# moss-lab/ScanFold

Hardware: AMD Instinct MI355X
Metric: windows/sec (W=120, step=1, 100 shuffles) (higher is better)
Workload: dtype int32 (int16 LDS storage) energies; f64 partition function

## Files before the change

### scanfold_amd/csrc/sf_mfe_fast.hip.h

```cpp
#pragma once
#include <type_traits>
#ifdef SF_EMUL
#include <vector>
#endif
#include "sf_energy.h"
#include "sf_pk16.h"

#define SF_FAST_NR 34
#ifndef SF_FAST_TINY_D0
#define SF_FAST_TINY_D0 10
#endif
#define SF_FAST_CHUNK_D0 36
#ifndef SF_FAST_SHORT
#define SF_FAST_SHORT 1
#endif
#ifndef SF_FAST_SHORT_D1
#define SF_FAST_SHORT_D1 18
#endif
#ifndef SF_FAST_SHORT_D2
#define SF_FAST_SHORT_D2 26
#endif
#define SF_FAST_SHORT_D3 32
#ifndef SF_FAST_UNPACK
#define SF_FAST_UNPACK 1
#endif
#ifndef SF_UNP_PB
#define SF_UNP_PB 4
#endif
#define SF_HELP_MERGE_MAXW 118
#define SF_DML_HELPER_BIAS_256 26
#define SF_DML_HELPER_BIAS_W200 50
#define SF_DML_HELPER_BIAS(ng, wt) ((ng) == 256 ? ((wt) == 200 ? SF_DML_HELPER_BIAS_W200 : SF_DML_HELPER_BIAS_256) : 100000)
#define SF_HELP_NB_128 4
#define SF_HELP_NB_128G 8
#define SF_HELP_NB_256 6
#define SF_INF16 30000
#define SF_FAST_THRESH 10000
#define SF_FAST_OVF (-12000)
#define SF_FAST_MAXPARAM 2500
#define SF_FAST_MAXW 256
#define SF_FAST_BIG 60000
#ifndef SF_FAST_WAVES_PER_SIMD
#define SF_FAST_WAVES_PER_SIMD 4
#endif

struct SfFastParams {
  int32_t NIN[32];
  int32_t IL[32];
  int32_t L1N[32];
  int32_t BUL[32];
  int32_t L23;
  int32_t fast_ok;
  int16_t mmI[200], mm1n[200], mm23[200], mmM[200], mmH[200], mmExt[200];
  int16_t stack[64];
  int16_t d5[40], d3[40];
  uint8_t pair[64];
  uint8_t rpair[64];
  int16_t stackT[64], mm23in[200];
  int16_t int11T[8 * 8 * 25], int21a[8 * 8 * 125], int21b[8 * 8 * 125], int22T[8 * 8 * 625];
  int16_t uni[128];
  int16_t uniG[31][128];
};
// ... 252 lines not shown
  if (q < sf_emul_span_lo || q + 2 * n16 > sf_emul_span_hi) {
    fprintf(stderr, "sf_mfe_fast (emulation): read for loop size %d, absent on diagonal %d, outside the rolling tables and their mirror rows (%ld bytes past their end)\n",
            u, d, (long)(q + 2 * n16 - sf_emul_span_hi));
    abort();
  }
  for (int k = 0; k < n16; k++) {
    const int s = sf_emul_shadow[(size_t)(q - sf_emul_span_lo) / 2 + k];
    if (s != 0) {
      fprintf(stderr, "sf_mfe_fast (emulation): read for loop size %d, absent on diagonal %d, finds an entry %s (entry %ld of the rolling tables)\n",
              u, d, s == 1 ? "a diagonal of this fold has written" : "this fold's prologue has not initialised", (long)((q - sf_emul_span_lo) / 2 + k));
      abort();
    }
  }
}
extern "C" int sfemul_absent_check_selftest(int W, int what) {
  const SfFastLayout L = sf_fast_layout(W);
  static std::vector<char> lds;
  lds.assign((size_t)L.total, 0);
  sf_emul_shadow_span(lds.data() + L.off_ci, lds.data() + L.off_tab);
  sf_emul_shadow_set(lds.data() + L.off_ci, (L.off_tab - L.off_ci) / 2, 0);
  if (what == 0) {
    const int16_t *e = (const int16_t *)(lds.data() + L.off_ci) + 3 * (W - 4) + 3;
    sf_emul_check_absent(e, 1, 10, 5);
    sf_emul_shadow_set(e, 1, 1);
    sf_emul_check_absent(e, 1, 10, 5);
  } else {
    sf_emul_check_absent(lds.data() + L.off_tab - 4, 2, 10, 8);
    sf_emul_check_absent(lds.data() + L.off_tab, 2, 10, 8);
  }
  return 0;
}
#define SF_EMUL_WROTE(p, n16) sf_emul_shadow_set((p), (n16), 1)
#define SF_EMUL_ABSENT(CHK, p, n16, d, u) do { if ((CHK) && (u) > (d) - 2 - (SFD_TURN + 1)) sf_emul_check_absent((p), (n16), (d), (u)); } while (0)
#else
#define SF_EMUL_WROTE(p, n16) ((void)0)
#define SF_EMUL_ABSENT(CHK, p, n16, d, u) ((void)0)
#endif

__device__ __forceinline__ void sf_fast_publish_bn(int16_t *w, const int i0, const uint32_t bn) {
  w[0] = (int16_t)sf_lo(bn);
  if (i0 > 0) w[-1] = (int16_t)sf_hi(bn);
  SF_EMUL_WROTE(w, 1);
  if (i0 > 0) SF_EMUL_WROTE(w - 1, 1);
}

enum { SF_SEC_P1 = 1, SF_SEC_HELP = 2, SF_SEC_DML = 4, SF_SEC_FIN = 8, SF_SEC_C0 = 16, SF_SEC_ALL = 31, SF_SEC_PRE = 32,
       SF_SEC_POST = 64 };
struct SfHU {
  short v[27];
};
struct SfPub {
  uint32_t a;
  uint32_t b;
  int tau;
  int type;
};
template <bool G, int WT, int SEC, bool CH = false, bool FOLD = false, int UCAP = SFD_MAXLOOP, int TBLK = 1, bool MGH = false,
          bool UNP = false, bool SHORT = false>
__device__ __forceinline__ void sf_fast_cell(const SfFastCtx &X, const int d, const int i, const bool valid,
                                             const int slot2, const int slotd, uint32_t (&HP)[14], SfHU &HU, int &ovf,
                                             const bool final_fml, const int fnb, int &fpart, int &dec, int &eh, int &e0,
                                             int &dprev, SfPub &pub, const int dml_lo = SFD_TURN + 1,
                                             const int dml_hi = 1 << 20) {
  const SfFastParams *const Fc = FOLD ? X.F : sf_const_base(X.F);
  const int16_t *const ubase = G ? X.uNIN : (CH ? Fc->uniG[sfd_max(sfd_min(d - 2 - (SFD_TURN + 1), 30), 0)] : Fc->uni);
  const int16_t *const uNIN = ubase, *const uIL = ubase + 32, *const uBN = ubase + 64;
#define CBAT(x) X.BN[2 * (x)]
#define C1NAT(x) X.BN[2 * ((x) - 1) + 1]
#define HGET(x) (((x)&1) ? ((int)HP[(x) >> 1] >> 16) : (int)(int16_t)(HP[(x) >> 1] & 0xffffu))
#define HSET(x, v)                                                                                       \
  HP[(x) >> 1] = ((x)&1) ? ((HP[(x) >> 1] & 0x0000ffffu) | ((uint32_t)(v) << 16))                         \
                         : ((HP[(x) >> 1] & 0xffff0000u) | ((uint32_t)(v)&0xffffu))
  const int W = WT ? WT : X.W, RW = W - 4;
  if (!valid) return;
  const int j = i + d, i0 = i - 1;
  const uint8_t *S = X.S;
  const int umax = G ? sfd_min(SFD_MAXLOOP, d - 2 - (SFD_TURN + 1)) : SFD_MAXLOOP;
  const int um = CH ? d - 2 - (SFD_TURN + 1) : SFD_MAXLOOP;
  int type = (SEC & SF_SEC_POST) ? pub.type : (d <= X.maxd ? X.tPair[S[i] * 8 + S[j]] : 0);
  if (!(SEC & SF_SEC_POST) && X.hc.c) {
    type = sf_hc_type_of(X.hc, type, i, j, d <= X.maxd);
    if (type == 7) { type = 0; ovf = 1; }
  }
  const int si1 = S[i + 1], sj1 = S[j - 1];
  if (SEC & SF_SEC_PRE) pub.type = type;
  if ((SEC & SF_SEC_PRE) && type) {
    const int tr = X.tRPair[S[i] * 8 + S[j]];
    const int sp1 = S[i - 1], sq1 = S[j + 1];
    const int tau_in = tr > 2 ? X.TAU : 0;
    int stem, ext;
    if (i > 1 && j < W) { stem = X.tM[SF_TIDX(type, sp1, sq1)]; ext = X.tE[SF_TIDX(type, sp1, sq1)]; }
    else if (i > 1) stem = ext = X.tD5[type * 5 + sp1];
    else if (j < W) stem = ext = X.tD3[type * 5 + sq1];
    else stem = ext = 0;
    pub.a = sf_pk(X.tI[SF_TIDX(tr, sq1, sp1)], X.t1n[SF_TIDX(tr, sq1, sp1)]);
    pub.b = sf_pk(stem + tau_in + X.MLintern, ext + tau_in);
    pub.tau = tau_in;
  }
#define FBASE(dd) (FOLD ? ((dd) <= (W + 3) / 2 ? ((dd)-4) * (W - 3) : (W - 1 - (dd)) * (W - 3) + (dd)-3) \
                        : (((dd)-4) * W - ((dd) * ((dd)-1) / 2 - 6) + (((dd)-4 + (W & 1)) >> 1)))
#define FLEN(dd) (W - (dd) + ((W - (dd)) & 1))
#define ROW(u) ((slot2 - (u) < 0 ? slot2 - (u) + SF_FAST_NR : slot2 - (u)) * RW)
  constexpr bool TBL = !G && TBLK != 0;
  constexpr int UTOP = (!G && UCAP < SFD_MAXLOOP) ? UCAP : SFD_MAXLOOP;
  constexpr bool UNG = !G && !CH;
  const SfFastRows *const Rc = TBL ? sf_const_base(X.R) : X.R;
  const int32_t *const rci_o = Rc->ci_odd[slot2], *const rci_e = Rc->ci_even[slot2];
  const int32_t *const rbn_o = Rc->bn_odd[slot2], *const rbn_e = Rc->bn_even[slot2];
#define ROWB_CI(u) (TBL ? (((u)&1) ? rci_o[(u) >> 1] : rci_e[(u) >> 1]) : 2 * ROW(u))
#define ROWB_BN(u) (TBL ? (((u)&1) ? rbn_o[(u) >> 1] : rbn_e[(u) >> 1]) : 4 * ROW(u))
#define CIROW(u) ((const int16_t *)((const char *)X.CI + ROWB_CI(u)))

  if (SEC & SF_SEC_P1) {
  if (UNP) {
    static_assert(!UNP || (!G && !CH && !FOLD), "the unpacked recurrence exists for the all-sizes code of the narrow kernel only");
    const int32_t *const nin = Fc->NIN;
    static_assert(!UNP || UTOP >= 7, "the unpacked recurrence keeps at least the sizes 6 and 7");
    short r30a = 0, r30b = 0;
    if (UTOP >= 30) {
      const int16_t *row = CIROW(30) + i0;
      SF_EMUL_ABSENT(true, row + 3, 1, d, 30); SF_EMUL_ABSENT(true, row + 29, 1, d, 30);
      r30a = row[3]; r30b = row[29];
    }
    constexpr int PB = SF_UNP_PB;
#pragma unroll
    for (int pb = 12; pb >= 1; pb -= PB) {
      short a3[PB], au[PB], b3[PB], bu[PB];
#pragma unroll
      for (int k = 0; k < PB; k++) {
// ... 304 lines not shown
          uint32_t ggp = sf_pk(32767, 32767);
#pragma unroll
          for (int pp = 1; pp <= 13; pp++)
            if (!CH || um >= 2 * pp + 4) ggp = sf_pkmin(ggp, sf_pkadd(HP[pp], sf_ldw(uIL + 2 * pp + 4)));
          gg = sfd_min(sf_lo(ggp), sf_hi(ggp));
        }
        e = sfd_min(e, gg + X.tI[SF_TIDX(type, si1, sj1)]);
      }
      {
        const int tr = X.tRPair[S[i] * 8 + S[j]];
        const int dml = dprev;
        e = sfd_min(e, dml + X.tM[SF_TIDX(tr, sj1, si1)] + (tr > 2 ? TAU : 0) + X.MLintern + X.MLclosing);
      }
      e0 = e;
    }
  }
  if ((SEC & SF_SEC_DML) && !(SEC & SF_SEC_FIN)) multiloop_split();

  if (!(SEC & SF_SEC_FIN)) return;
  int c = SF_INF16;
  if (type) {
    c = sfd_min(e0, eh);
    if (c < SF_FAST_OVF) ovf = 1;
  }

  const int rbd = slotd * RW + i0;
  int f = SF_FAST_BIG, cx = SF_INF16;
  if (SEC & SF_SEC_POST) {
    X.CI[rbd] = (int16_t)(c + sf_lo(pub.a));
    if (!FOLD && slotd == 0) X.CI[SF_FAST_NR * RW + i0] = (int16_t)(c + sf_lo(pub.a));
    const uint32_t bn = sf_pk(c + pub.tau, c + sf_hi(pub.a));
    sf_fast_publish_bn(X.BN + 2 * rbd, i0, bn);
    if (X.bn_dup && slotd == 0) sf_fast_publish_bn(X.BN + 2 * (SF_FAST_NR * RW + i0), i0, bn);
    f = c + sf_lo(pub.b);
    cx = sfd_min(c + sf_hi(pub.b), SF_INF16);
  } else if (type) {
    const int tr = X.tRPair[S[i] * 8 + S[j]];
    const int sp1 = S[i - 1], sq1 = S[j + 1];
    const int tau_in = tr > 2 ? X.TAU : 0;
    X.CI[rbd] = (int16_t)(c + X.tI[SF_TIDX(tr, sq1, sp1)]);
    if (!FOLD && slotd == 0) X.CI[SF_FAST_NR * RW + i0] = X.CI[rbd];
    const uint32_t bn = sf_pk(c + tau_in, c + X.t1n[SF_TIDX(tr, sq1, sp1)]);
    sf_fast_publish_bn(X.BN + 2 * rbd, i0, bn);
    if (X.bn_dup && slotd == 0) sf_fast_publish_bn(X.BN + 2 * (SF_FAST_NR * RW + i0), i0, bn);
    int stem, ext;
    if (i > 1 && j < W) { stem = X.tM[SF_TIDX(type, sp1, sq1)]; ext = X.tE[SF_TIDX(type, sp1, sq1)]; }
    else if (i > 1) stem = ext = X.tD5[type * 5 + sp1];
    else if (j < W) stem = ext = X.tD3[type * 5 + sq1];
    else stem = ext = 0;
    f = c + stem + tau_in + X.MLintern;
    cx = sfd_min(c + ext + tau_in, SF_INF16);
  } else {
    X.CI[rbd] = SF_INF16; sf_fast_publish_bn(X.BN + 2 * rbd, i0, sf_pk(SF_INF16, SF_INF16));
    if (!FOLD && slotd == 0) X.CI[SF_FAST_NR * RW + i0] = SF_INF16;
    if (X.bn_dup && slotd == 0) sf_fast_publish_bn(X.BN + 2 * (SF_FAST_NR * RW + i0), i0, sf_pk(SF_INF16, SF_INF16));
  }
  SF_EMUL_WROTE(X.CI + rbd, 1);
  if (!FOLD && slotd == 0) SF_EMUL_WROTE(X.CI + SF_FAST_NR * RW + i0, 1);
  X.cg[SF_CGIDX(i, j)] = (int16_t)cx;
  if (final_fml && d > SFD_TURN + 1) f = sfd_min(f, fnb);
  if ((SEC & SF_SEC_DML) && (SEC & SF_SEC_FIN)) multiloop_split();
  f = sfd_min(f, dec);
  dprev = dec > SF_FAST_THRESH ? SF_INF16 : dec;
  fpart = f;
  if (final_fml && f < SF_FAST_OVF) ovf = 1;
  X.fML[FBASE(d) + i0] = (int16_t)(f > SF_FAST_THRESH ? SF_INF16 : f);
#undef ROW
#undef ROWB_CI
#undef ROWB_BN
#undef CIROW
#undef BNROWB
}

__device__ __forceinline__ int sf_wave_min(int v) {
#ifdef SF_EMUL
  return sfemul_wave_min(v);
#else
  v = sfd_min(v, __builtin_amdgcn_update_dpp(v, v, 0xB1, 0xF, 0xF, false));
  v = sfd_min(v, __builtin_amdgcn_update_dpp(v, v, 0x4E, 0xF, 0xF, false));
  v = sfd_min(v, __builtin_amdgcn_update_dpp(v, v, 0x141, 0xF, 0xF, false));
  v = sfd_min(v, __builtin_amdgcn_update_dpp(v, v, 0x140, 0xF, 0xF, false));
  v = sfd_min(v, __builtin_amdgcn_update_dpp(v, v, 0x142, 0xA, 0xF, false));
  v = sfd_min(v, __builtin_amdgcn_update_dpp(v, v, 0x143, 0xC, 0xF, false));
  return __builtin_amdgcn_readlane(v, 63);
#endif
}

__device__ __forceinline__ uint32_t sf_wave_next(uint32_t v) {
#ifdef SF_EMUL
  return __shfl_down(v, 1);
#else
  return (uint32_t)__builtin_amdgcn_update_dpp(0, (int)v, 0x130, 0xF, 0xF, true);
#endif
}

template <int WT, int LGC = 0>
__device__ __forceinline__ int sf_fast_dml2(const SfFastCtx &X, const int d, const int lane, const int i_own, const bool valid) {
  constexpr bool FOLD = false;
  const int W = WT ? WT : X.W;
// ... 264 lines not shown
            }
          }
        }
        }
        load_row(i + PF, cb[k]);
      }
    }
  }
  for (int jf = sfd_max(W - SFD_TURN - 1, 1); jf <= W; jf++) {
    f5prev = sfd_min(f5prev, column_min(jf));
    if (want_trace && lane == 0) f5s[jf] = f5prev;
  }
  SF_WAVE_SYNC();
  const int over = flag[0] || f5prev < SF_FAST_OVF;
  if (lane == 0) {
    out[seq] = f5prev;
    if (over) {
      const int k = atomicAdd(ovf_cnt, 1);
      ovf_list[k] = seq;
    }
  }
  if (db_out && !over && (seq % trace_stride) == 0) {
    int16_t *stI = stack_area;
    int16_t *stJ = stI + W + 8;
    int16_t *stM = stJ + W + 8;
    const int bad = sf_fast_traceback(X, f5s, tExt, lane, stI, stJ, stM, dbL);
    char *dst = db_out + (size_t)(seq / trace_stride) * (W + 1);
    for (int x = lane; x <= W; x += 64) dst[x] = x < W ? dbL[x] : 0;
    if (bad && lane == 0) atomicOr(status, 1);
  }
}

#define SF_DEFER_ROWS_256 3
template <int NQ>
struct SfTrail {
  int F[NQ];
  int f3n;
  int row;
};
template <int NQ>
__device__ __forceinline__ void sf_trail_load(const int16_t *cgp, const int W, const int lane, const int i, int (&c)[NQ]) {
#pragma unroll
  for (int q = 0; q < NQ; q++) {
    const int j = lane + 1 + 64 * q;
    c[q] = (i >= 1 && j <= W && i + SFD_TURN + 1 <= j) ? (int)cgp[SF_CGIDX(i, j)] : SF_INF16;
  }
}
template <int NQ>
__device__ __forceinline__ void sf_trail_row(SfTrail<NQ> &T, const int lane, const int i, const int (&c)[NQ]) {
  if (i < 1) return;
  int m = c[0] + T.F[0];
#pragma unroll
  for (int q = 1; q < NQ; q++) m = sfd_min(m, c[q] + T.F[q]);
  T.f3n = sfd_min(T.f3n, sf_wave_min(m));
  if (i >= 2) {
    const int l = (i - 2) & 63, h = (i - 2) >> 6;
#pragma unroll
    for (int q = 0; q < NQ; q++) T.F[q] = (lane == l && h == q) ? T.f3n : T.F[q];
  }
}
template <int NQ, int NR>
__device__ __forceinline__ void sf_trail_rows(SfTrail<NQ> &T, const int lane, const int nrows, const int (&c)[NR][NQ]) {
#pragma unroll
  for (int k = 0; k < NR; k++)
    if (k < nrows) sf_trail_row<NQ>(T, lane, T.row - k, c[k]);
  T.row -= nrows;
// ... 62 lines not shown
  uint8_t *const hcP = (uint8_t *)hcC + (W + 2), *const hcE = hcP + (W + 2);
  int16_t *const scS = (int16_t *)(smem + Lo.off_hc + (((3 * (W + 2)) + 1) & ~1));
  X.hc.c = (HC && cons_rows) ? hcC : nullptr; X.hc.partner = hcP; X.hc.encl = hcE;
  X.sc = (HC && sc_rows) ? scS : nullptr;
  X.fML = (int16_t *)smem;
  X.CI = (int16_t *)(smem + Lo.off_ci);
  X.C1N = nullptr; X.CB = nullptr;
  X.BN = (int16_t *)(smem + Lo.off_c1n);
#ifdef SF_EMUL
  sf_emul_bn_base = (const char *)X.BN; sf_emul_ci_base = (const char *)X.CI;
  sf_emul_shadow_span((const char *)(smem + Lo.off_ci), (const char *)(smem + Lo.off_tab));
#endif
  X.DMLr = nullptr;
  int16_t *tab = (int16_t *)(smem + Lo.off_tab);
  X.t23 = tab; X.tI = tab + 175 - 25; X.t1n = tab + 325 - 25; X.tM = tab + 475 - 25; X.tH = tab + 625 - 25;
  X.tE = tab + 775 - 25; X.cg_ext = 1;
  X.tStack = tab + 925; X.tD5 = tab + 989; X.tD3 = tab + 1029;
  uint8_t *tPair = (uint8_t *)(tab + 1069);
  X.tPair = tPair;
  uint8_t *tRPair = (uint8_t *)(tab + SF_FAST_TAB_OLD);
  int16_t *t23in = tab + SF_FAST_TAB_OLD + 32;
  X.tRPair = tRPair; X.t23in = t23in;
  int32_t *flag = (int32_t *)(smem + Lo.off_flag);
  uint8_t *S = (uint8_t *)(smem + Lo.off_S);
  X.S = S;
  X.D = D; X.F = F; X.R = Rows; X.W = W; X.fold = FOLD; X.maxd = D->max_pair_dist;
  constexpr bool MERGE = MG && (NG == 128);
  constexpr bool UNPK = SF_FAST_UNPACK && (NG == 128);
  constexpr bool SHORTU = SF_FAST_SHORT && UNPK && !HC;
  static_assert(SF_FAST_TINY_D0 >= 10 && SF_FAST_TINY_D0 <= SF_FAST_SHORT_D1 && SF_FAST_SHORT_D1 <= SF_FAST_SHORT_D2 &&
                SF_FAST_SHORT_D2 <= SF_FAST_SHORT_D3 && SF_FAST_SHORT_D1 >= 14, "SHORT loops: d0 >= 10 (no tabulated hairpin, sizes 0 .. 4 exist), caps >= 7");
  constexpr bool LGLOOPS = MG && (NG == 128);
  constexpr bool ROLE_LOOPS = (NG == 128);
  constexpr int TBLK = WT > 0 ? 1 : (NG == 128 ? (MG ? 2 : 1) : 0);
  X.bn_dup = (NG == 128);
  uint8_t *const cell_list = (MG && W >= SF_HELP_MERGE_MAXW) ? (uint8_t *)((int16_t *)(smem + Lo.off_tab) + 1069 + 32 + 1)
                                                            : (uint8_t *)(smem + Lo.off_list);
  X.TAU = D->P.TerminalAU; X.MLbase = D->P.MLbase; X.MLclosing = D->P.MLclosing; X.MLintern = D->P.MLintern[1];
  int32_t *f5s = (int32_t *)(smem + Lo.off_ci);
  int16_t *tExt = (int16_t *)(smem + Lo.off_ci + (((W + 1) * 4 + 3) & ~3));

  const int tid = threadIdx.x;
  X.cg = cg_all + (size_t)sf_fast_scratch_slot(blockIdx.x, gridDim.x) * SF_CG_ENTRIES(W);
  for (int x = tid; x < 175; x += NT) {
    tab[x] = F->mm23[x];
    if (x < 150) {
      tab[175 + x] = F->mmI[25 + x]; tab[325 + x] = F->mm1n[25 + x]; tab[475 + x] = F->mmM[25 + x];
      tab[625 + x] = F->mmH[25 + x]; tab[775 + x] = F->mmExt[25 + x];
    }
  }
  for (int x = tid; x < 175; x += NT) t23in[x] = F->mm23in[x];
  for (int x = tid; x < 64; x += NT) { tab[925 + x] = F->stackT[x]; tPair[x] = F->pair[x]; tRPair[x] = F->rpair[x]; }
  for (int x = tid; x < 40; x += NT) { tab[989 + x] = F->d5[x]; tab[1029 + x] = F->d3[x]; }

  {
    int16_t *uni = tab + 1069 + 32 + 1;
    X.uNIN = uni;
    for (int x = tid; x < 128; x += NT) uni[x] = F->uni[x];
  }
  const int grp = SF_WAVE_UNIFORM(tid / NG);
  const int tg = tid - grp * NG;
  constexpr int CENTRE = (NG == 256) ? 128 : 32;
  constexpr bool SHARE = SF_DML_HELPER_BIAS(NG, WT) < 10000;
  constexpr bool DML2 = (NG == 128);
  const int OFFs = ((W + 1) >> 1) - CENTRE;
  const int OFF = (NG > 64) ? (OFFs + NG) & (NG - 1) : 0;
// ... 66 lines not shown
    const bool trail_this = defer_on && !(db_out && (seq % trace_stride) == 0);
    if (sweeper) {
#pragma unroll
      for (int q = 0; q < NQ; q++) T.F[q] = 0;
      T.f3n = 0; T.row = trail_this ? W - SFD_TURN - 1 : 0;
    }
    int ovf = 0;
    uint32_t H[14];
    int dprev = SF_INF16;
    int fnb = SF_FAST_BIG;
#pragma unroll
    for (int k = 0; k < 14; k++) H[k] = (uint32_t)SF_INF16 | ((uint32_t)SF_INF16 << 16);

    int slot2 = (SFD_TURN + 1 + grp - 2) % SF_FAST_NR, slotd = (SFD_TURN + 1 + grp) % SF_FAST_NR;
    auto build_list = [&](const int dd0) {
      const int lane = tid & 63;
      const int d1 = dd0 + 1;
      const int iH = ((v - 64) & (NG - 1)) - (dd0 >> 1);
      const bool vA = (dd0 < W) && (iH >= 1) && (iH + dd0 <= W), vB = (d1 < W) && (iH >= 1) && (iH + d1 <= W);
      const int tA = (vA && dd0 <= X.maxd) ? X.tPair[S[iH] * 8 + S[iH + dd0]] : 0;
      const int tB = (vB && d1 <= X.maxd) ? X.tPair[S[iH] * 8 + S[iH + d1]] : 0;
      const unsigned long long mA = __ballot(tA != 0), mB = __ballot(tB != 0);
      const int cA = __popcll(mA);
      uint8_t *list = cell_list + (((dd0 >> 1) & 1) << 7);
      const unsigned long long below = (1ull << lane) - 1ull;
      if (tA) list[__popcll(mA & below)] = (uint8_t)iH;
      if (tB) list[cA + __popcll(mB & below)] = (uint8_t)(iH | 128);
      if (lane == 0) list[127] = (uint8_t)(cA + __popcll(mB));
      if (lane == 0) SF_EMUL_WROTE(list, 64);
    };
    SfHU HU;
    const int grp_wave = grp;
    const bool sweeper_wave = sweeper;
    auto step = [&](const int d0, auto kind_tag, auto role_tag) {
      constexpr SfStep KIND = decltype(kind_tag)::value;
      constexpr SfRole ROLE = decltype(role_tag)::value;
      constexpr bool ROLES = ROLE != SF_ROLE_ALL;
      static_assert(!ROLES || (NG == 128 && KIND >= SF_STEP_SPLIT && KIND <= SF_STEP_SPLIT8), "roles: the narrow kernel's split steps");
      const int grp = ROLES ? (int)(ROLE == SF_ROLE_MAIN_ODD || ROLE == SF_ROLE_HELP_ODD) : grp_wave;
      const bool hwave = ROLES ? ROLE >= SF_ROLE_HELP_EVEN : tg >= 64;
      const bool sweeper = ROLES ? ROLE == SF_ROLE_HELP_ODD : sweeper_wave;
      constexpr int LGC = KIND == SF_STEP_SPLIT16 ? 4 : (KIND == SF_STEP_SPLIT8 ? 3 : (KIND == SF_STEP_SPLIT && LGLOOPS ? 5 : 0));
      constexpr bool DO_G = KIND == SF_STEP_SIZED, DO_CH = KIND == SF_STEP_GUARDED;
      const int d = d0 + grp;
      constexpr bool DO_SH = KIND >= SF_STEP_SHORT_A && KIND <= SF_STEP_SHORT_C;
      constexpr int SHCAP = KIND == SF_STEP_SHORT_A ? SF_FAST_SHORT_D1 - 7 : (KIND == SF_STEP_SHORT_B ? SF_FAST_SHORT_D2 - 7 : SFD_MAXLOOP);
      if (!ROLES && d0 == SFD_TURN + 1 + 2 && tid == 0) *next_slot = fetched;
      if (!ROLES && d0 == SFD_TURN + 1 + 4) next_seq = SF_WAVE_UNIFORM(*next_slot);
      constexpr bool split = KIND >= SF_STEP_SPLIT;
      constexpr bool narrow = KIND == SF_STEP_NARROW;
      if (NARROW && d0 == narrow_d0) {
        uint32_t *const xa = (uint32_t *)X.BN;
        const int RWc = W - 4;
        if (tg >= 96 && tg < 160) {
#pragma unroll
          for (int k = 0; k < 14; k++) xa[(grp * 16 + k) * RWc + 100 + (tg - 96)] = H[k];
          xa[(grp * 16 + 14) * RWc + 100 + (tg - 96)] = (uint32_t)dprev;
          xa[(grp * 16 + 15) * RWc + 100 + (tg - 96)] = (uint32_t)fnb;
        }
        __syncthreads();
        if (tg >= 64 && tg < 128) {
#pragma unroll
          for (int k = 0; k < 14; k++) H[k] = xa[(grp * 16 + k) * RWc + 100 + (tg - 64)];
          dprev = (int)xa[(grp * 16 + 14) * RWc + 100 + (tg - 64)];
          fnb = (int)xa[(grp * 16 + 15) * RWc + 100 + (tg - 64)];
        }
        __syncthreads();
      }
      const bool helper = split && (NG == 256 ? (narrow ? tg < 64 : (tg < 64 || tg >= 192)) : hwave);
      const int vh = NG == 256 ? (narrow ? v + 96 : (tg < 64 ? v + 64 : v - 64)) : v - 64;
      const int vm = narrow ? ((v + 32) & (NG - 1)) : v;
      constexpr bool DML4 = NARROW && (WT == 200);
      const bool dmlw = DML4 && narrow && tg >= 128;
      const int vd = tg >= 192 ? v - 96 : v - 32;
      const int i = (NARROW && !DML4 && narrow && tg >= 128) ? -1
                    : ((dmlw ? (vd & (NG - 1)) : (helper ? (vh & (NG - 1)) : vm)) - (d >> 1));
      const int dml_terms = d - 2 * SFD_TURN - 2;
      const int dml_cut = d - SFD_TURN - 1 - sfd_max(sfd_min(dml_terms / 2 - SF_DML_HELPER_BIAS(NG, WT), dml_terms), 0);
      const bool valid = (d < W) && (i >= 1) && (i + d <= W);
      int fpart = SF_FAST_BIG;
      int dec = SF_FAST_BIG, eh = SF_FAST_BIG, e0 = SF_FAST_BIG;
      SfPub pub;
      pub.a = pub.b = 0; pub.tau = 0; pub.type = 0;
      int dc[DROWS][NQ];
      const bool sweep_now = defer_on && sweeper && split && T.row > 0;
      const int sweep_rows = sweep_now ? sfd_max(sfd_min(defer_rows, T.row - (W - d0)), 0) : 0;
      if (sweep_now) {
#pragma unroll
        for (int k = 0; k < DROWS; k++)
          if (k < sweep_rows) sf_trail_load<NQ>(X.cg, W, tid & 63, T.row - k, dc[k]);
      }
      if (__ballot(valid)) {
        if (DO_G && d0 < 8) sf_fast_cell<true, WT, SF_SEC_ALL, false, FOLD, 1>(X, d, i, valid, slot2, slotd, H, HU, ovf, grp == 0, fnb, fpart, dec, eh, e0, dprev, pub);
        else if (DO_G && d0 < SF_FAST_TINY_D0) sf_fast_cell<true, WT, SF_SEC_ALL, false, FOLD, 5>(X, d, i, valid, slot2, slotd, H, HU, ovf, grp == 0, fnb, fpart, dec, eh, e0, dprev, pub);
        else if (DO_CH && d0 < SF_FAST_CHUNK_D0) sf_fast_cell<false, WT, SF_SEC_ALL, true, FOLD, SFD_MAXLOOP, TBLK>(X, d, i, valid, slot2, slotd, H, HU, ovf, grp == 0, fnb, fpart, dec, eh, e0, dprev, pub);
        else if (DO_SH) sf_fast_cell<false, WT, SF_SEC_ALL, false, FOLD, SHORTU ? SHCAP : SFD_MAXLOOP, TBLK, false, SHORTU, SHORTU>(X, d, i, valid, slot2, slotd, H, HU, ovf, grp == 0, fnb, fpart, dec, eh, e0, dprev, pub);
        else if (!split) sf_fast_cell<false, WT, SF_SEC_ALL, false, FOLD, SFD_MAXLOOP, TBLK, false, UNPK && KIND == SF_STEP_UNSPLIT>(X, d, i, valid, slot2, slotd, H, HU, ovf, grp == 0, fnb, fpart, dec, eh, e0, dprev, pub);
        else if (DML4 && narrow) {
          const int nmain = dml_terms / 5, cA = SFD_TURN + 1 + nmain, cB = cA + (dml_terms - nmain + 1) / 2;
          uint32_t *const xa = (uint32_t *)X.BN;
          if (dmlw) {
            const bool wB = tg >= 192;
            sf_fast_cell<false, WT, SF_SEC_DML, false, FOLD, SFD_MAXLOOP, TBLK>(X, d, i, valid, slot2, slotd, H, HU, ovf, false, fnb, fpart, dec, eh, e0, dprev, pub, wB ? cB : cA, wB ? (1 << 20) : cB - 1);
            if (valid) xa[(grp * 16 + (wB ? 1 : 0)) * (W - 4) + 100 + (tg & 63)] = (uint32_t)sfd_min(dec, 32000);
          } else if (!helper) {
            sf_fast_cell<false, WT, SF_SEC_P1 | SF_SEC_C0 | SF_SEC_DML | SF_SEC_PRE, false, FOLD, SFD_MAXLOOP, TBLK>(X, d, i, valid, slot2, slotd, H, HU, ovf, grp == 0, fnb, fpart, dec, eh, e0, dprev, pub, SFD_TURN + 1, cA - 1);
          } else {
            sf_fast_cell<false, WT, SF_SEC_HELP, false, FOLD, SFD_MAXLOOP, TBLK>(X, d, i, valid, slot2, slotd, H, HU, ovf, grp == 0, fnb, fpart, dec, eh, e0, dprev, pub);
            if (valid) X.BN[2 * (slotd * (W - 4) + i - 1)] = (int16_t)sfd_min(eh, 32000);
          }
        }
        else if (!helper) {
          if (SHARE) sf_fast_cell<false, WT, SF_SEC_P1 | SF_SEC_C0 | SF_SEC_DML | SF_SEC_PRE, false, FOLD, SFD_MAXLOOP, TBLK>(X, d, i, valid, slot2, slotd, H, HU, ovf, grp == 0, fnb, fpart, dec, eh, e0, dprev, pub, SFD_TURN + 1, dml_cut - 1);
          else {
            static_assert(SHARE || DML2, "a main wave either shares the multiloop split with its helpers (NG = 256) or runs it two cells per lane (NG = 128)");
            dec = sf_fast_dml2<WT, LGC>(X, d, tid & 63, i, valid);
            sf_fast_cell<false, WT, SF_SEC_P1 | SF_SEC_C0 | SF_SEC_PRE, false, FOLD, SFD_MAXLOOP, TBLK, false, UNPK && split>(X, d, i, valid, slot2, slotd, H, HU, ovf, grp == 0, fnb, fpart, dec, eh, e0, dprev, pub);
          }
        } else if (MERGE) {
          const int lane = tid & 63;
          const uint8_t *list = cell_list + (((d0 >> 1) & 1) << 7);
          const int cT = SF_WAVE_UNIFORM((int)list[127]);
          const int e = (grp << 6) + lane;
          if (SF_WAVE_UNIFORM(cT > (grp << 6))) {
            const bool vC = e < cT;
            const int ent = vC ? list[e] : 1;
            const int g = ent >> 7, iC = ent & 127;
            const int s2 = slot2 - grp < 0 ? slot2 - grp + SF_FAST_NR : slot2 - grp;
            const int sd0 = slotd - grp < 0 ? slotd - grp + SF_FAST_NR : slotd - grp;
            const int sd1 = sd0 + 1 >= SF_FAST_NR ? 0 : sd0 + 1;
            SfFastCtx Xh = X;
            Xh.BN = X.BN + 2 * g * (W - 4);
            sf_fast_cell<false, WT, SF_SEC_HELP, false, FOLD, SFD_MAXLOOP, TBLK, true>(Xh, d0 + g, iC, vC, s2, sd0, H, HU, ovf, false, fnb, fpart, dec, eh, e0, dprev, pub);
            if (vC) { X.BN[2 * ((g ? sd1 : sd0) * (W - 4) + iC - 1)] = (int16_t)sfd_min(eh, 32000); SF_EMUL_WROTE(X.BN + 2 * ((g ? sd1 : sd0) * (W - 4) + iC - 1), 1); }
          }
        } else {
          if (SHARE) {
            sf_fast_cell<false, WT, SF_SEC_HELP | SF_SEC_DML, false, FOLD, SFD_MAXLOOP, TBLK>(X, d, i, valid, slot2, slotd, H, HU, ovf, grp == 0, fnb, fpart, dec, eh, e0, dprev, pub, dml_cut);
            if (valid) {
              X.BN[2 * (slotd * (W - 4) + i - 1)] = (int16_t)sfd_min(eh, 32000);
              X.CI[slotd * (W - 4) + i - 1] = (int16_t)sfd_min(dec, 32000);
            }
          } else {
            sf_fast_cell<false, WT, SF_SEC_HELP, false, FOLD, SFD_MAXLOOP, TBLK>(X, d, i, valid, slot2, slotd, H, HU, ovf, grp == 0, fnb, fpart, dec, eh, e0, dprev, pub);
            if (valid) { X.BN[2 * (slotd * (W - 4) + i - 1)] = (int16_t)sfd_min(eh, 32000); SF_EMUL_WROTE(X.BN + 2 * (slotd * (W - 4) + i - 1), 1); }
          }
        }
      }
      if (sweep_now && sweep_rows > 0) sf_trail_rows<NQ, DROWS>(T, tid & 63, sweep_rows, dc);
      if (MERGE && grp == 1 && hwave && (ROLES || d0 + 2 >= split_d0) && d0 + 2 < W) build_list(d0 + 2);
      if (split) {
        __syncthreads();
        if (!helper && !dmlw && __ballot(valid)) {
          if (valid) {
            eh = X.BN[2 * (slotd * (W - 4) + i - 1)];
            if (DML4 && narrow) {
              const uint32_t *const xa = (const uint32_t *)X.BN;
              dec = sfd_min(dec, sfd_min((int)xa[(grp * 16) * (W - 4) + 100 + (tg & 63)], (int)xa[(grp * 16 + 1) * (W - 4) + 100 + (tg & 63)]));
            } else if (SHARE) dec = sfd_min(dec, (int)X.CI[slotd * (W - 4) + i - 1]);
          }
          sf_fast_cell<false, WT, SF_SEC_FIN | SF_SEC_POST, false, FOLD, SFD_MAXLOOP, TBLK>(X, d, i, valid, slot2, slotd, H, HU, ovf, grp == 0, fnb, fpart, dec, eh, e0, dprev, pub);
        }
      }
      __syncthreads();
      if (grp == 0 && valid && !helper && !dmlw) {
        const int d1 = d0 + 1;
        const int16_t *pd = X.fML + FBASE(d1), *pe = X.fML + FBASE(d0);
        const bool ex0 = i + d1 <= W, ex1 = i >= 2;
        const int ia = i - 1, ib = ex1 ? i - 2 : 0;
        const int p0 = pd[ia], p1 = pd[ib], q0 = pe[i], q1 = pe[ia], q2 = pe[ib];
        const int v0 = sfd_min(p0, sfd_min(q0, q1) + X.MLbase), v1 = sfd_min(p1, sfd_min(q1, q2) + X.MLbase);
        if ((ex0 && v0 < SF_FAST_OVF) || (ex1 && v1 < SF_FAST_OVF)) ovf = 1;
        const int g0 = (ex0 && v0 <= SF_FAST_THRESH) ? v0 : SF_INF16, g1 = (ex1 && v1 <= SF_FAST_THRESH) ? v1 : SF_INF16;
        if (ex0) X.fML[FBASE(d1) + ia] = (int16_t)g0;
        fnb = sfd_min(g0, g1) + X.MLbase;
      }
      slot2 += 2; if (slot2 >= SF_FAST_NR) slot2 -= SF_FAST_NR;
      slotd += 2; if (slotd >= SF_FAST_NR) slotd -= SF_FAST_NR;
    };
    {
      int d0 = SFD_TURN + 1;
      constexpr SfRoleTag<SF_ROLE_ALL> all_roles{};
      auto unpack_state = [&]() {
#pragma unroll
        for (int x = 0; x < 27; x++) HU.v[x] = (short)((x & 1) ? (H[x >> 1] >> 16) : (H[x >> 1] & 0xffffu));
      };
      for (; d0 < SF_FAST_TINY_D0 && d0 < W; d0 += 2) step(d0, SfStepTag<SF_STEP_SIZED>{}, all_roles);
      if constexpr (SHORTU) {
        unpack_state();
        for (; d0 < SF_FAST_SHORT_D1 && d0 < W; d0 += 2) step(d0, SfStepTag<SF_STEP_SHORT_A>{}, all_roles);
        for (; d0 < SF_FAST_SHORT_D2 && d0 < W; d0 += 2) step(d0, SfStepTag<SF_STEP_SHORT_B>{}, all_roles);
        for (; d0 < SF_FAST_SHORT_D3 && d0 < W; d0 += 2) step(d0, SfStepTag<SF_STEP_SHORT_C>{}, all_roles);
      } else {
        for (; d0 < SF_FAST_CHUNK_D0 && d0 < W; d0 += 2) step(d0, SfStepTag<SF_STEP_GUARDED>{}, all_roles);
        if constexpr (UNPK) unpack_state();
      }
      for (; d0 < split_d0 && d0 < W; d0 += 2) step(d0, SfStepTag<SF_STEP_UNSPLIT>{}, all_roles);
      auto split_loops = [&](auto role_tag) {
        if constexpr (LGLOOPS) {
          for (; d0 < W - 30 && d0 < W; d0 += 2) step(d0, SfStepTag<SF_STEP_SPLIT>{}, role_tag);
          for (; d0 < W - 14 && d0 < W; d0 += 2) step(d0, SfStepTag<SF_STEP_SPLIT16>{}, role_tag);
          for (; d0 < W; d0 += 2) step(d0, SfStepTag<SF_STEP_SPLIT8>{}, role_tag);
        }
        for (; d0 < W; d0 += 2) step(d0, SfStepTag<SF_STEP_SPLIT>{}, role_tag);
      };
      if constexpr (ROLE_LOOPS) {
        const int wave = SF_WAVE_UNIFORM(tid >> 6);
        if (wave == 0) split_loops(SfRoleTag<SF_ROLE_MAIN_EVEN>{});
        else if (wave == 2) split_loops(SfRoleTag<SF_ROLE_MAIN_ODD>{});
        else if (wave == 1) split_loops(SfRoleTag<SF_ROLE_HELP_EVEN>{});
        else split_loops(SfRoleTag<SF_ROLE_HELP_ODD>{});
        if (wave != 3) {
#pragma unroll
          for (int q = 0; q < NQ; q++) T.F[q] = 0;
          T.f3n = 0; T.row = 0;
        }
      } else {
        for (; d0 < (NARROW ? narrow_d0 : W) && d0 < W; d0 += 2) step(d0, SfStepTag<SF_STEP_SPLIT>{}, all_roles);
      }
      if constexpr (NARROW)
        for (; d0 < W; d0 += 2) step(d0, SfStepTag<SF_STEP_NARROW>{}, all_roles);
    }

    if (ovf) flag[0] = 1;
    if (trail_this) {
      __syncthreads();
      if (sweeper) {
        while (T.row >= 1) {
          int tc[4][NQ];
#pragma unroll
          for (int k = 0; k < 4; k++) sf_trail_load<NQ>(X.cg, W, tid & 63, T.row - k, tc[k]);
// ... 80 lines not shown
```

Baseline: 47210.

## Move exterior-loop term lookups to helper waves and carry fML diagonal base

In the split diagonal loops with NG=128, helper waves now compute the pair's stem/ext and interior terms (SF_SEC_TERMS) and hand them to the main wave through LDS scratch in BN/CI/fML. This takes table lookups off the main wave's critical path. The fML diagonal base offset is now carried incrementally in a scalar instead of being recomputed with the quadratic FBASE formula each step. For W=120, sweep row counts are specialised per loop kind. The cost is extra LDS writes and reads for the hand-over, and a dependence on enough free room in the BN rows.

```diff
diff --git a/scanfold_amd/csrc/sf_mfe_fast.hip.h b/scanfold_amd/csrc/sf_mfe_fast.hip.h
--- a/scanfold_amd/csrc/sf_mfe_fast.hip.h
+++ b/scanfold_amd/csrc/sf_mfe_fast.hip.h
@@ -28,6 +28,12 @@
 #define SF_UNP_PB 4
 #endif
 #define SF_HELP_MERGE_MAXW 118
+#ifndef SF_FAST_HELPER_TERMS
+#define SF_FAST_HELPER_TERMS 1
+#endif
+#ifndef SF_FAST_FBASE_CARRY
+#define SF_FAST_FBASE_CARRY 1
+#endif
 #define SF_DML_HELPER_BIAS_256 26
 #define SF_DML_HELPER_BIAS_W200 50
 #define SF_DML_HELPER_BIAS(ng, wt) ((ng) == 256 ? ((wt) == 200 ? SF_DML_HELPER_BIAS_W200 : SF_DML_HELPER_BIAS_256) : 100000)
@@ -346,9 +352,13 @@
 }
 #define SF_EMUL_WROTE(p, n16) sf_emul_shadow_set((p), (n16), 1)
 #define SF_EMUL_ABSENT(CHK, p, n16, d, u) do { if ((CHK) && (u) > (d) - 2 - (SFD_TURN + 1)) sf_emul_check_absent((p), (n16), (d), (u)); } while (0)
+#define SF_LOCKSTEP() ((void)__ballot(1))
+#define SF_PIN_S(x) ((void)0)
 #else
 #define SF_EMUL_WROTE(p, n16) ((void)0)
 #define SF_EMUL_ABSENT(CHK, p, n16, d, u) ((void)0)
+#define SF_LOCKSTEP() ((void)0)
+#define SF_PIN_S(x) asm volatile("" : "+s"(x))
 #endif
 
 __device__ __forceinline__ void sf_fast_publish_bn(int16_t *w, const int i0, const uint32_t bn) {
@@ -359,7 +369,7 @@
 }
 
 enum { SF_SEC_P1 = 1, SF_SEC_HELP = 2, SF_SEC_DML = 4, SF_SEC_FIN = 8, SF_SEC_C0 = 16, SF_SEC_ALL = 31, SF_SEC_PRE = 32,
-       SF_SEC_POST = 64 };
+       SF_SEC_POST = 64, SF_SEC_TERMS = 128, SF_SEC_TYPE = 256, SF_SEC_XTERMS = 512, SF_SEC_FB = 1024 };
 struct SfHU {
   short v[27];
 };
@@ -368,6 +378,7 @@
   uint32_t b;
   int tau;
   int type;
+  int stem, ext;
 };
 template <bool G, int WT, int SEC, bool CH = false, bool FOLD = false, int UCAP = SFD_MAXLOOP, int TBLK = 1, bool MGH = false,
           bool UNP = false, bool SHORT = false>
@@ -375,7 +386,7 @@
                                              const int slot2, const int slotd, uint32_t (&HP)[14], SfHU &HU, int &ovf,
                                              const bool final_fml, const int fnb, int &fpart, int &dec, int &eh, int &e0,
                                              int &dprev, SfPub &pub, const int dml_lo = SFD_TURN + 1,
-                                             const int dml_hi = 1 << 20) {
+                                             const int dml_hi = 1 << 20, const int fbd = 0) {
   const SfFastParams *const Fc = FOLD ? X.F : sf_const_base(X.F);
   const int16_t *const ubase = G ? X.uNIN : (CH ? Fc->uniG[sfd_max(sfd_min(d - 2 - (SFD_TURN + 1), 30), 0)] : Fc->uni);
   const int16_t *const uNIN = ubase, *const uIL = ubase + 32, *const uBN = ubase + 64;
@@ -397,18 +408,27 @@
     if (type == 7) { type = 0; ovf = 1; }
   }
   const int si1 = S[i + 1], sj1 = S[j - 1];
-  if (SEC & SF_SEC_PRE) pub.type = type;
-  if ((SEC & SF_SEC_PRE) && type) {
+  if (SEC & (SF_SEC_PRE | SF_SEC_TYPE)) pub.type = type;
+  if (SEC & SF_SEC_TYPE) pub.tau = type > 2 ? X.TAU : 0;
+  if ((SEC & (SF_SEC_PRE | SF_SEC_TERMS)) && type) {
     const int tr = X.tRPair[S[i] * 8 + S[j]];
     const int sp1 = S[i - 1], sq1 = S[j + 1];
     const int tau_in = tr > 2 ? X.TAU : 0;
     int stem, ext;
+    if (SEC & SF_SEC_TERMS) {
+      const int km = SF_TIDX(type, sp1, sq1);
+      const int mm = X.tM[km], me = X.tE[km], e5 = X.tD5[type * 5 + sp1], e3 = X.tD3[type * 5 + sq1];
+      const bool in5 = i > 1, in3 = j < W;
+      const int dg = in5 ? e5 : (in3 ? e3 : 0);
+      stem = (in5 && in3) ? mm : dg; ext = (in5 && in3) ? me : dg;
+    } else
     if (i > 1 && j < W) { stem = X.tM[SF_TIDX(type, sp1, sq1)]; ext = X.tE[SF_TIDX(type, sp1, sq1)]; }
     else if (i > 1) stem = ext = X.tD5[type * 5 + sp1];
     else if (j < W) stem = ext = X.tD3[type * 5 + sq1];
     else stem = ext = 0;
     pub.a = sf_pk(X.tI[SF_TIDX(tr, sq1, sp1)], X.t1n[SF_TIDX(tr, sq1, sp1)]);
-    pub.b = sf_pk(stem + tau_in + X.MLintern, ext + tau_in);
+    if (SEC & SF_SEC_TERMS) { pub.stem = stem + tau_in + X.MLintern; pub.ext = ext + tau_in; }
+    else pub.b = sf_pk(stem + tau_in + X.MLintern, ext + tau_in);
     pub.tau = tau_in;
   }
 #define FBASE(dd) (FOLD ? ((dd) <= (W + 3) / 2 ? ((dd)-4) * (W - 3) : (W - 1 - (dd)) * (W - 3) + (dd)-3) \
@@ -779,8 +799,8 @@
     const uint32_t bn = sf_pk(c + pub.tau, c + sf_hi(pub.a));
     sf_fast_publish_bn(X.BN + 2 * rbd, i0, bn);
     if (X.bn_dup && slotd == 0) sf_fast_publish_bn(X.BN + 2 * (SF_FAST_NR * RW + i0), i0, bn);
-    f = c + sf_lo(pub.b);
-    cx = sfd_min(c + sf_hi(pub.b), SF_INF16);
+    f = c + ((SEC & SF_SEC_XTERMS) ? pub.stem : sf_lo(pub.b));
+    cx = sfd_min(c + ((SEC & SF_SEC_XTERMS) ? pub.ext : sf_hi(pub.b)), SF_INF16);
   } else if (type) {
     const int tr = X.tRPair[S[i] * 8 + S[j]];
     const int sp1 = S[i - 1], sq1 = S[j + 1];
@@ -811,7 +831,7 @@
   dprev = dec > SF_FAST_THRESH ? SF_INF16 : dec;
   fpart = f;
   if (final_fml && f < SF_FAST_OVF) ovf = 1;
-  X.fML[FBASE(d) + i0] = (int16_t)(f > SF_FAST_THRESH ? SF_INF16 : f);
+  X.fML[((SEC & SF_SEC_FB) ? fbd : FBASE(d)) + i0] = (int16_t)(f > SF_FAST_THRESH ? SF_INF16 : f);
 #undef ROW
 #undef ROWB_CI
 #undef ROWB_BN
@@ -1142,6 +1162,11 @@
 }
 
 #define SF_DEFER_ROWS_256 3
+#ifndef SF_SWEEP_ROWS_120_A
+#define SF_SWEEP_ROWS_120_A 4
+#define SF_SWEEP_ROWS_120_B 4
+#define SF_SWEEP_ROWS_120_C 4
+#endif
 template <int NQ>
 struct SfTrail {
   int F[NQ];
@@ -1270,6 +1295,8 @@
                 SF_FAST_SHORT_D2 <= SF_FAST_SHORT_D3 && SF_FAST_SHORT_D1 >= 14, "SHORT loops: d0 >= 10 (no tabulated hairpin, sizes 0 .. 4 exist), caps >= 7");
   constexpr bool LGLOOPS = MG && (NG == 128);
   constexpr bool ROLE_LOOPS = (NG == 128);
+  constexpr bool HTERMS = SF_FAST_HELPER_TERMS && (NG == 128) && !HC;
+  constexpr bool FBCARRY = SF_FAST_FBASE_CARRY && (NG == 128) && !HC;
   constexpr int TBLK = WT > 0 ? 1 : (NG == 128 ? (MG ? 2 : 1) : 0);
   X.bn_dup = (NG == 128);
   uint8_t *const cell_list = (MG && W >= SF_HELP_MERGE_MAXW) ? (uint8_t *)((int16_t *)(smem + Lo.off_tab) + 1069 + 32 + 1)
@@ -1402,6 +1429,7 @@
     SfHU HU;
     const int grp_wave = grp;
     const bool sweeper_wave = sweeper;
+    int fb0 = 0;
     auto step = [&](const int d0, auto kind_tag, auto role_tag) {
       constexpr SfStep KIND = decltype(kind_tag)::value;
       constexpr SfRole ROLE = decltype(role_tag)::value;
@@ -1419,6 +1447,27 @@
       if (!ROLES && d0 == SFD_TURN + 1 + 4) next_seq = SF_WAVE_UNIFORM(*next_slot);
       constexpr bool split = KIND >= SF_STEP_SPLIT;
       constexpr bool narrow = KIND == SF_STEP_NARROW;
+      constexpr bool HT = HTERMS && split && ROLES && LGLOOPS && KIND == SF_STEP_SPLIT, FB = FBCARRY && split && ROLES;
+      constexpr int SEC_MAIN = SF_SEC_P1 | SF_SEC_C0 | (HT ? SF_SEC_TYPE : SF_SEC_PRE);
+      constexpr int SEC_HELP = SF_SEC_HELP | (HT ? SF_SEC_TERMS : 0);
+      constexpr int SEC_FIN = SF_SEC_FIN | SF_SEC_POST | (HT ? SF_SEC_XTERMS : 0) | (FB ? SF_SEC_FB : 0);
+      int fbA = 0, fbB = 0;
+      if (HT || FB) {
+        fbA = FB ? fb0 : FBASE(d0);
+        fbB = FB ? fb0 + FLEN(d0) : FBASE(d0 + 1);
+        if (FB) SF_PIN_S(fbB);
+      }
+      const int fbd = grp ? fbB : fbA;
+      auto hand_over = [&](const int row, const int x, const int n, const int fb, const int eh_, const SfPub &p) {
+        *(uint32_t *)(X.BN + 2 * (row + x)) = p.a;
+        X.CI[row + x] = (int16_t)sfd_min(eh_, 32000);
+        X.fML[fb + x] = (int16_t)p.stem;
+        X.BN[2 * row + 2 * n + x] = (int16_t)p.ext;
+        SF_EMUL_WROTE(X.BN + 2 * (row + x), 2); SF_EMUL_WROTE(X.CI + row + x, 1); SF_EMUL_WROTE(X.BN + 2 * row + 2 * n + x, 1);
+      };
+#ifdef SF_EMUL
+      if (HT && d < W && 3 * (W - d) > 2 * (W - 4)) { fprintf(stderr, "sf_mfe_fast (emulation): W %d diagonal %d: no room for the helper's terms\n", W, d); abort(); }
+#endif
       if (NARROW && d0 == narrow_d0) {
         uint32_t *const xa = (uint32_t *)X.BN;
         const int RWc = W - 4;
@@ -1451,13 +1500,15 @@
       int fpart = SF_FAST_BIG;
       int dec = SF_FAST_BIG, eh = SF_FAST_BIG, e0 = SF_FAST_BIG;
       SfPub pub;
-      pub.a = pub.b = 0; pub.tau = 0; pub.type = 0;
-      int dc[DROWS][NQ];
+      pub.a = pub.b = 0; pub.tau = 0; pub.type = 0; pub.stem = pub.ext = 0;
+      constexpr bool SWK = (WT == 120) && ROLES;
+      constexpr int DR = !SWK ? DROWS : (KIND == SF_STEP_SPLIT ? SF_SWEEP_ROWS_120_A : (KIND == SF_STEP_SPLIT16 ? SF_SWEEP_ROWS_120_B : SF_SWEEP_ROWS_120_C));
+      int dc[DR][NQ];
       const bool sweep_now = defer_on && sweeper && split && T.row > 0;
-      const int sweep_rows = sweep_now ? sfd_max(sfd_min(defer_rows, T.row - (W - d0)), 0) : 0;
+      const int sweep_rows = sweep_now ? sfd_max(sfd_min(SWK ? DR : defer_rows, T.row - (W - d0)), 0) : 0;
       if (sweep_now) {
 #pragma unroll
-        for (int k = 0; k < DROWS; k++)
+        for (int k = 0; k < DR; k++)
           if (k < sweep_rows) sf_trail_load<NQ>(X.cg, W, tid & 63, T.row - k, dc[k]);
       }
       if (__ballot(valid)) {
@@ -1485,7 +1536,7 @@
           else {
             static_assert(SHARE || DML2, "a main wave either shares the multiloop split with its helpers (NG = 256) or runs it two cells per lane (NG = 128)");
             dec = sf_fast_dml2<WT, LGC>(X, d, tid & 63, i, valid);
-            sf_fast_cell<false, WT, SF_SEC_P1 | SF_SEC_C0 | SF_SEC_PRE, false, FOLD, SFD_MAXLOOP, TBLK, false, UNPK && split>(X, d, i, valid, slot2, slotd, H, HU, ovf, grp == 0, fnb, fpart, dec, eh, e0, dprev, pub);
+            sf_fast_cell<false, WT, SEC_MAIN, false, FOLD, SFD_MAXLOOP, TBLK, false, UNPK && split>(X, d, i, valid, slot2, slotd, H, HU, ovf, grp == 0, fnb, fpart, dec, eh, e0, dprev, pub);
           }
         } else if (MERGE) {
           const int lane = tid & 63;
@@ -1501,8 +1552,9 @@
             const int sd1 = sd0 + 1 >= SF_FAST_NR ? 0 : sd0 + 1;
             SfFastCtx Xh = X;
             Xh.BN = X.BN + 2 * g * (W - 4);
-            sf_fast_cell<false, WT, SF_SEC_HELP, false, FOLD, SFD_MAXLOOP, TBLK, true>(Xh, d0 + g, iC, vC, s2, sd0, H, HU, ovf, false, fnb, fpart, dec, eh, e0, dprev, pub);
-            if (vC) { X.BN[2 * ((g ? sd1 : sd0) * (W - 4) + iC - 1)] = (int16_t)sfd_min(eh, 32000); SF_EMUL_WROTE(X.BN + 2 * ((g ? sd1 : sd0) * (W - 4) + iC - 1), 1); }
+            sf_fast_cell<false, WT, SEC_HELP, false, FOLD, SFD_MAXLOOP, TBLK, true>(Xh, d0 + g, iC, vC, s2, sd0, H, HU, ovf, false, fnb, fpart, dec, eh, e0, dprev, pub);
+            if (vC && HT) hand_over((g ? sd1 : sd0) * (W - 4), iC - 1, W - d0 - g, g ? fbB : fbA, eh, pub);
+            else if (vC) { X.BN[2 * ((g ? sd1 : sd0) * (W - 4) + iC - 1)] = (int16_t)sfd_min(eh, 32000); SF_EMUL_WROTE(X.BN + 2 * ((g ? sd1 : sd0) * (W - 4) + iC - 1), 1); }
           }
         } else {
           if (SHARE) {
@@ -1512,39 +1564,48 @@
               X.CI[slotd * (W - 4) + i - 1] = (int16_t)sfd_min(dec, 32000);
             }
           } else {
-            sf_fast_cell<false, WT, SF_SEC_HELP, false, FOLD, SFD_MAXLOOP, TBLK>(X, d, i, valid, slot2, slotd, H, HU, ovf, grp == 0, fnb, fpart, dec, eh, e0, dprev, pub);
-            if (valid) { X.BN[2 * (slotd * (W - 4) + i - 1)] = (int16_t)sfd_min(eh, 32000); SF_EMUL_WROTE(X.BN + 2 * (slotd * (W - 4) + i - 1), 1); }
+            sf_fast_cell<false, WT, SEC_HELP, false, FOLD, SFD_MAXLOOP, TBLK>(X, d, i, valid, slot2, slotd, H, HU, ovf, grp == 0, fnb, fpart, dec, eh, e0, dprev, pub);
+            if (valid && HT) hand_over(slotd * (W - 4), i - 1, W - d, fbd, eh, pub);
+            else if (valid) { X.BN[2 * (slotd * (W - 4) + i - 1)] = (int16_t)sfd_min(eh, 32000); SF_EMUL_WROTE(X.BN + 2 * (slotd * (W - 4) + i - 1), 1); }
           }
         }
       }
-      if (sweep_now && sweep_rows > 0) sf_trail_rows<NQ, DROWS>(T, tid & 63, sweep_rows, dc);
+      if (sweep_now && sweep_rows > 0) sf_trail_rows<NQ, DR>(T, tid & 63, sweep_rows, dc);
       if (MERGE && grp == 1 && hwave && (ROLES || d0 + 2 >= split_d0) && d0 + 2 < W) build_list(d0 + 2);
       if (split) {
         __syncthreads();
         if (!helper && !dmlw && __ballot(valid)) {
-          if (valid) {
+          if (valid && HT) {
+            const int row = slotd * (W - 4), x = i - 1;
+            const uint32_t wa = sf_ldw(X.BN + 2 * (row + x));
+            const int te = X.CI[row + x], ts = X.fML[fbd + x], tx = X.BN[2 * row + 2 * (W - d) + x];
+            const bool tp = pub.type != 0;
+            eh = te; pub.a = tp ? wa : 0u; pub.stem = tp ? ts : 0; pub.ext = tp ? tx : 0;
+          } else if (valid) {
             eh = X.BN[2 * (slotd * (W - 4) + i - 1)];
             if (DML4 && narrow) {
               const uint32_t *const xa = (const uint32_t *)X.BN;
               dec = sfd_min(dec, sfd_min((int)xa[(grp * 16) * (W - 4) + 100 + (tg & 63)], (int)xa[(grp * 16 + 1) * (W - 4) + 100 + (tg & 63)]));
             } else if (SHARE) dec = sfd_min(dec, (int)X.CI[slotd * (W - 4) + i - 1]);
           }
-          sf_fast_cell<false, WT, SF_SEC_FIN | SF_SEC_POST, false, FOLD, SFD_MAXLOOP, TBLK>(X, d, i, valid, slot2, slotd, H, HU, ovf, grp == 0, fnb, fpart, dec, eh, e0, dprev, pub);
+          if (HT) SF_LOCKSTEP();
+          sf_fast_cell<false, WT, SEC_FIN, false, FOLD, SFD_MAXLOOP, TBLK>(X, d, i, valid, slot2, slotd, H, HU, ovf, grp == 0, fnb, fpart, dec, eh, e0, dprev, pub, SFD_TURN + 1, 1 << 20, fbd);
         }
       }
       __syncthreads();
       if (grp == 0 && valid && !helper && !dmlw) {
         const int d1 = d0 + 1;
-        const int16_t *pd = X.fML + FBASE(d1), *pe = X.fML + FBASE(d0);
+        const int16_t *pd = X.fML + (FB ? fbB : FBASE(d1)), *pe = X.fML + (FB ? fbA : FBASE(d0));
         const bool ex0 = i + d1 <= W, ex1 = i >= 2;
         const int ia = i - 1, ib = ex1 ? i - 2 : 0;
         const int p0 = pd[ia], p1 = pd[ib], q0 = pe[i], q1 = pe[ia], q2 = pe[ib];
         const int v0 = sfd_min(p0, sfd_min(q0, q1) + X.MLbase), v1 = sfd_min(p1, sfd_min(q1, q2) + X.MLbase);
         if ((ex0 && v0 < SF_FAST_OVF) || (ex1 && v1 < SF_FAST_OVF)) ovf = 1;
         const int g0 = (ex0 && v0 <= SF_FAST_THRESH) ? v0 : SF_INF16, g1 = (ex1 && v1 <= SF_FAST_THRESH) ? v1 : SF_INF16;
-        if (ex0) X.fML[FBASE(d1) + ia] = (int16_t)g0;
+        if (ex0) X.fML[(FB ? fbB : FBASE(d1)) + ia] = (int16_t)g0;
         fnb = sfd_min(g0, g1) + X.MLbase;
       }
+      if (FB) fb0 += 2 * (W - d0);
       slot2 += 2; if (slot2 >= SF_FAST_NR) slot2 -= SF_FAST_NR;
       slotd += 2; if (slotd >= SF_FAST_NR) slotd -= SF_FAST_NR;
     };
@@ -1567,6 +1628,7 @@
       }
       for (; d0 < split_d0 && d0 < W; d0 += 2) step(d0, SfStepTag<SF_STEP_UNSPLIT>{}, all_roles);
       auto split_loops = [&](auto role_tag) {
+        if constexpr (FBCARRY) fb0 = FBASE(d0);
         if constexpr (LGLOOPS) {
           for (; d0 < W - 30 && d0 < W; d0 += 2) step(d0, SfStepTag<SF_STEP_SPLIT>{}, role_tag);
           for (; d0 < W - 14 && d0 < W; d0 += 2) step(d0, SfStepTag<SF_STEP_SPLIT16>{}, role_tag);
```

Result: faster. 47880, median of 6 (+1.4%).
